# zifuwan/Sigma

Measured on AMD Instinct MI355X. Metric: images/sec fwd+bwd sigma_small 480x640, higher is better.
Workload: dtype f32

## Files before the change

### sigma_amd/csrc/layernorm.hip

```cpp
#include <hip/hip_runtime.h>
#include <stdint.h>

#include "../../include/sigma_ops.h"
#include "scan_device.h"

namespace sigma {

namespace {

__device__ __forceinline__ float wave_allsum(float v) { return wave_sum(v); }

struct LnArgs {
    const float* x; const float* gamma; const float* beta; const float* dy;
    float* y; float* mean; float* rstd; float* dx; float* ws;
    const float* z; float* dz; long z_stride, dz_stride;
    const float* rsc; long rows_per_scale;
    const float* dx_add;
    long M; int C; float eps;
};

__device__ __forceinline__ float sigmoid_f(float v) {
    return __builtin_amdgcn_rcpf(1.0f + __builtin_amdgcn_exp2f(-v * 1.4426950408889634f));
}

template <int NV>
__global__ void __launch_bounds__(256) ln_fwd_kernel(const LnArgs a) {
    const int lane = threadIdx.x & 63;
    const long wave = (long)blockIdx.x * 4 + (threadIdx.x >> 6);
    const long nwaves = (long)gridDim.x * 4;
    const int C = a.C;
    float4 g[NV], b[NV];
#pragma unroll
    for (int j = 0; j < NV; ++j) {
        const int c = lane * 4 + 256 * j;
        g[j] = c < C ? *reinterpret_cast<const float4*>(a.gamma + c) : make_float4(0, 0, 0, 0);
        b[j] = (c < C && a.beta) ? *reinterpret_cast<const float4*>(a.beta + c) : make_float4(0, 0, 0, 0);
    }
    const float inv = 1.0f / (float)C;
    long sb = a.rsc ? wave / a.rows_per_scale : 0, srem = a.rsc ? wave - sb * a.rows_per_scale : 0;
    const bool gatedf = a.z != nullptr;
    auto load_row = [&](long r, float4 (&xv)[NV], float4 (&zv)[NV]) {
        const float* __restrict__ xr = a.x + r * C;
#pragma unroll
        for (int j = 0; j < NV; ++j) {
            const int c = lane * 4 + 256 * j;
            xv[j] = c < C ? *reinterpret_cast<const float4*>(xr + c) : make_float4(0, 0, 0, 0);
            zv[j] = (gatedf && c < C) ? *reinterpret_cast<const float4*>(a.z + r * a.z_stride + c) : make_float4(0, 0, 0, 0);
        }
    };
    constexpr bool kPrefetch = NV <= 2;
    float4 v[NV], zc[NV];
    if (kPrefetch && wave < a.M) load_row(wave, v, zc);
    for (long r = wave; r < a.M; r += nwaves) {
        if (!kPrefetch) load_row(r, v, zc);
        float4 vn[NV], zn[NV];
        const bool more = kPrefetch && r + nwaves < a.M;
        if (more) load_row(r + nwaves, vn, zn);
        float s = 0.0f;
#pragma unroll
        for (int j = 0; j < NV; ++j) s += (v[j].x + v[j].y) + (v[j].z + v[j].w);
        const float mu = wave_allsum(s) * inv;
        float q = 0.0f;
#pragma unroll
        for (int j = 0; j < NV; ++j) {
            const int c = lane * 4 + 256 * j;
            if (c < C) {
                const float dx0 = v[j].x - mu, dx1 = v[j].y - mu, dx2 = v[j].z - mu, dx3 = v[j].w - mu;
                q += (dx0 * dx0 + dx1 * dx1) + (dx2 * dx2 + dx3 * dx3);
            }
        }
        const float rs = rsqrtf(wave_allsum(q) * inv + a.eps);
        float* __restrict__ yr = a.y + r * C;
        float sc = 1.0f;
        if (a.rsc) {
            sc = a.rsc[sb];
            srem += nwaves;
            while (srem >= a.rows_per_scale) { srem -= a.rows_per_scale; ++sb; }
        }
#pragma unroll
        for (int j = 0; j < NV; ++j) {
            const int c = lane * 4 + 256 * j;
            if (c < C) {
                float4 o;
                o.x = (v[j].x - mu) * rs * g[j].x + b[j].x;
                o.y = (v[j].y - mu) * rs * g[j].y + b[j].y;
                o.z = (v[j].z - mu) * rs * g[j].z + b[j].z;
                o.w = (v[j].w - mu) * rs * g[j].w + b[j].w;
                if (gatedf) {
                    const float4 zv = zc[j];
                    o.x *= zv.x * sigmoid_f(zv.x); o.y *= zv.y * sigmoid_f(zv.y);
                    o.z *= zv.z * sigmoid_f(zv.z); o.w *= zv.w * sigmoid_f(zv.w);
                }
                if (a.rsc) { o.x *= sc; o.y *= sc; o.z *= sc; o.w *= sc; }
                *reinterpret_cast<float4*>(yr + c) = o;
            }
        }
        if (lane == 0 && a.mean) { a.mean[r] = mu; a.rstd[r] = rs; }
        if (more) {
#pragma unroll
            for (int j = 0; j < NV; ++j) { v[j] = vn[j]; zc[j] = zn[j]; }
        }
    }
}

template <int NV>
__global__ void __launch_bounds__(256) ln_bwd_kernel(const LnArgs a) {
    const int lane = threadIdx.x & 63;
    const long wave = (long)blockIdx.x * 4 + (threadIdx.x >> 6);
    const long nwaves = (long)gridDim.x * 4;
    const int C = a.C;
    float4 g[NV], dg[NV], db[NV];
#pragma unroll
    for (int j = 0; j < NV; ++j) {
        const int c = lane * 4 + 256 * j;
        g[j] = c < C ? *reinterpret_cast<const float4*>(a.gamma + c) : make_float4(0, 0, 0, 0);
        dg[j] = make_float4(0, 0, 0, 0);
        db[j] = make_float4(0, 0, 0, 0);
    }
    const bool gated = a.z != nullptr;
    const float inv = 1.0f / (float)C;
    long sb = a.rsc ? wave / a.rows_per_scale : 0, srem = a.rsc ? wave - sb * a.rows_per_scale : 0;
    auto load_row = [&](long r, float4 (&xv)[NV], float4 (&gv)[NV], float4 (&zv)[NV], float& mu, float& rs) {
        const float* __restrict__ xr = a.x + r * C;
        const float* __restrict__ gr = a.dy + r * C;
        mu = a.mean[r]; rs = a.rstd[r];
#pragma unroll
        for (int j = 0; j < NV; ++j) {
            const int c = lane * 4 + 256 * j;
            const bool in = c < C;
            xv[j] = in ? *reinterpret_cast<const float4*>(xr + c) : make_float4(0, 0, 0, 0);
            gv[j] = in ? *reinterpret_cast<const float4*>(gr + c) : make_float4(0, 0, 0, 0);
            zv[j] = (gated && in) ? *reinterpret_cast<const float4*>(a.z + r * a.z_stride + c) : make_float4(0, 0, 0, 0);
        }
    };
    float4 bv_[NV];
#pragma unroll
    for (int j = 0; j < NV; ++j) {
        const int c = lane * 4 + 256 * j;
        bv_[j] = (gated && a.beta && c < C) ? *reinterpret_cast<const float4*>(a.beta + c) : make_float4(0, 0, 0, 0);
    }
    constexpr bool kPrefetch = NV <= 2;
    float4 xc[NV], gc[NV], zc[NV];
    float mu = 0.0f, rs = 0.0f;
    if (kPrefetch && wave < a.M) load_row(wave, xc, gc, zc, mu, rs);
    for (long r = wave; r < a.M; r += nwaves) {
        if (!kPrefetch) load_row(r, xc, gc, zc, mu, rs);
        float4 xn[NV], gn[NV], zn[NV];
        float mun = 0.0f, rsn = 0.0f;
        const bool more = kPrefetch && r + nwaves < a.M;
        if (more) load_row(r + nwaves, xn, gn, zn, mun, rsn);
        float sc = 1.0f;
        if (a.rsc) {
            sc = a.rsc[sb];
            srem += nwaves;
            while (srem >= a.rows_per_scale) { srem -= a.rows_per_scale; ++sb; }
        }
        float4 xh[NV], t[NV];
        float s1 = 0.0f, s2 = 0.0f;
#pragma unroll
        for (int j = 0; j < NV; ++j) {
            const int c = lane * 4 + 256 * j;
            if (c < C) {
                const float4 xv = xc[j];
                float4 gv = gc[j];
                if (a.rsc) { gv.x *= sc; gv.y *= sc; gv.z *= sc; gv.w *= sc; }
                xh[j] = make_float4((xv.x - mu) * rs, (xv.y - mu) * rs, (xv.z - mu) * rs, (xv.w - mu) * rs);
                if (gated) {
                    const float4 zv = zc[j];
                    const float4 bv = bv_[j];
                    const float s0 = sigmoid_f(zv.x), s1_ = sigmoid_f(zv.y), s2_ = sigmoid_f(zv.z), s3 = sigmoid_f(zv.w);
                    float4 dzv;
                    dzv.x = gv.x * fmaf(xh[j].x, g[j].x, bv.x) * s0 * fmaf(zv.x, 1.0f - s0, 1.0f);
                    dzv.y = gv.y * fmaf(xh[j].y, g[j].y, bv.y) * s1_ * fmaf(zv.y, 1.0f - s1_, 1.0f);
                    dzv.z = gv.z * fmaf(xh[j].z, g[j].z, bv.z) * s2_ * fmaf(zv.z, 1.0f - s2_, 1.0f);
                    dzv.w = gv.w * fmaf(xh[j].w, g[j].w, bv.w) * s3 * fmaf(zv.w, 1.0f - s3, 1.0f);
                    *reinterpret_cast<float4*>(a.dz + r * a.dz_stride + c) = dzv;
                    gv.x *= zv.x * s0; gv.y *= zv.y * s1_; gv.z *= zv.z * s2_; gv.w *= zv.w * s3;
                }
                t[j] = make_float4(gv.x * g[j].x, gv.y * g[j].y, gv.z * g[j].z, gv.w * g[j].w);
                s1 += (t[j].x + t[j].y) + (t[j].z + t[j].w);
                s2 += (t[j].x * xh[j].x + t[j].y * xh[j].y) + (t[j].z * xh[j].z + t[j].w * xh[j].w);
                dg[j].x += gv.x * xh[j].x; dg[j].y += gv.y * xh[j].y; dg[j].z += gv.z * xh[j].z; dg[j].w += gv.w * xh[j].w;
                db[j].x += gv.x; db[j].y += gv.y; db[j].z += gv.z; db[j].w += gv.w;
            } else {
                xh[j] = make_float4(0, 0, 0, 0);
                t[j] = make_float4(0, 0, 0, 0);
            }
        }
        const float m1 = wave_allsum(s1) * inv, m2 = wave_allsum(s2) * inv;
        float* __restrict__ dr = a.dx + r * C;
        const float* __restrict__ ar = a.dx_add ? a.dx_add + r * C : nullptr;
#pragma unroll
        for (int j = 0; j < NV; ++j) {
            const int c = lane * 4 + 256 * j;
            if (c < C) {
                float4 o;
                o.x = rs * (t[j].x - m1 - xh[j].x * m2);
                o.y = rs * (t[j].y - m1 - xh[j].y * m2);
                o.z = rs * (t[j].z - m1 - xh[j].z * m2);
                o.w = rs * (t[j].w - m1 - xh[j].w * m2);
                if (ar) {
                    const float4 e = *reinterpret_cast<const float4*>(ar + c);
                    o.x += e.x; o.y += e.y; o.z += e.z; o.w += e.w;
                }
                *reinterpret_cast<float4*>(dr + c) = o;
            }
        }
        if (more) {
#pragma unroll
            for (int j = 0; j < NV; ++j) { xc[j] = xn[j]; gc[j] = gn[j]; zc[j] = zn[j]; }
            mu = mun; rs = rsn;
        }
    }
    extern __shared__ float part[];
    const int wv = threadIdx.x >> 6;
#pragma unroll
    for (int j = 0; j < NV; ++j) {
        const int c = lane * 4 + 256 * j;
        if (c < C) {
            *reinterpret_cast<float4*>(part + (wv * 2 + 0) * C + c) = dg[j];
            *reinterpret_cast<float4*>(part + (wv * 2 + 1) * C + c) = db[j];
        }
    }
    __syncthreads();
    float* __restrict__ wrow = a.ws + (long)blockIdx.x * 2 * C;
    for (int i = threadIdx.x * 4; i < 2 * C; i += 1024) {
        const float4 p0 = *reinterpret_cast<const float4*>(part + i), p1 = *reinterpret_cast<const float4*>(part + 2 * C + i);
        const float4 p2 = *reinterpret_cast<const float4*>(part + 4 * C + i), p3 = *reinterpret_cast<const float4*>(part + 6 * C + i);
        *reinterpret_cast<float4*>(wrow + i) = make_float4((p0.x + p1.x) + (p2.x + p3.x), (p0.y + p1.y) + (p2.y + p3.y),
                                                          (p0.z + p1.z) + (p2.z + p3.z), (p0.w + p1.w) + (p2.w + p3.w));
    }
}

__global__ void __launch_bounds__(256) ln_reduce_kernel(const float* __restrict__ ws, float* __restrict__ dgamma,
                                                        float* __restrict__ dbeta, int nwaves, int C) {
    __shared__ float red[16][17];
    const int tx = threadIdx.x & 15, ty = threadIdx.x >> 4;
    const int i = blockIdx.x * 16 + tx;
    const bool live = i < 2 * C;
    const int which = live ? i / C : 0, c = live ? i - which * C : 0;
    const float* __restrict__ col = ws + (long)which * C + c;
    const long stride = 2L * C;
    float a0 = 0.0f, a1 = 0.0f, a2 = 0.0f, a3 = 0.0f;
    if (live) {
        int w = ty;
        for (; w + 48 < nwaves; w += 64) {
            a0 += col[(long)w * stride];
            a1 += col[(long)(w + 16) * stride];
            a2 += col[(long)(w + 32) * stride];
            a3 += col[(long)(w + 48) * stride];
        }
        for (; w < nwaves; w += 16) a0 += col[(long)w * stride];
    }
    red[ty][tx] = (a0 + a1) + (a2 + a3);
    __syncthreads();
    if (ty == 0 && live) {
        float acc = 0.0f;
#pragma unroll
        for (int k = 0; k < 16; ++k) acc += red[k][tx];
        if (which == 0) dgamma[c] = acc;
        else if (dbeta) dbeta[c] = acc;
    }
}

template <typename F>
bool dispatch_nv(int C, F&& f) {
    const int nv = (C + 255) / 256;
    switch (nv) {
        case 1: f(std::integral_constant<int, 1>()); return true;
        case 2: f(std::integral_constant<int, 2>()); return true;
        case 3: f(std::integral_constant<int, 3>()); return true;
        case 4: f(std::integral_constant<int, 4>()); return true;
        case 5: case 6: f(std::integral_constant<int, 6>()); return true;
        case 7: case 8: f(std::integral_constant<int, 8>()); return true;
        default: return false;
    }
}

int grid_blocks(long M, long cap = 2048) {
    long b = (M + 3) / 4;
    if (b > cap) b = cap;
    if (b < 1) b = 1;
    return (int)b;
}
constexpr long kBwdBlocks = 512;
long bwd_blocks(long rows, int C) {
    long cap = (2L << 20) / (8L * C);
    if (cap > 2048) cap = 2048;
    if (cap < kBwdBlocks) cap = kBwdBlocks;
    return cap;
}

template <int NV, bool BWD>
int resident_blocks() {
    static int cached = 0;
    if (cached == 0) {
        int n = 0;
        hipError_t e = BWD ? hipOccupancyMaxActiveBlocksPerMultiprocessor(&n, ln_bwd_kernel<NV>, 256, 8 * 256 * NV * sizeof(float))
                           : hipOccupancyMaxActiveBlocksPerMultiprocessor(&n, ln_fwd_kernel<NV>, 256, 0);
        cached = (e == hipSuccess && n > 0) ? (n > 8 ? 8 : n) : 4;
    }
    return cached;
}

int fwd_grid(long rows, int C) {
    int occ = 8;
    dispatch_nv(C, [&](auto nv) { occ = resident_blocks<decltype(nv)::value, false>(); });
    return grid_blocks(rows, 256L * occ);
}

int bwd_grid(long rows, int C) {
    int occ = 8;
    dispatch_nv(C, [&](auto nv) { occ = resident_blocks<decltype(nv)::value, true>(); });
    long cap = bwd_blocks(rows, C);
    if (cap > 256L * occ) cap = 256L * occ;
    return grid_blocks(rows, cap);
}

bool check(const sigma_layernorm_params* p) {
    return p && p->rows >= 0 && p->channels > 0 && p->channels % 4 == 0 && p->channels <= 2048;
}

}

}

extern "C" {

int sigma_layernorm_bwd_partial_rows(int64_t rows, int32_t channels) {
    return sigma::bwd_grid(rows, channels > 0 ? channels : 4);
}

int sigma_layernorm_fwd(const sigma_layernorm_params* p, void* stream) {
    if (!sigma::check(p)) return SIGMA_OPS_ERR_ARG;
    if (p->rows == 0) return SIGMA_OPS_OK;
    if (!p->x || !p->gamma || !p->y) return SIGMA_OPS_ERR_ARG;
    sigma::LnArgs a{};
    a.x = p->x; a.gamma = p->gamma; a.beta = p->beta; a.y = p->y; a.mean = p->mean; a.rstd = p->rstd;
    a.z = p->gate; a.z_stride = p->gate_row_stride;
    if (p->gate && (p->gate_row_stride % 4 != 0 || p->gate_row_stride < p->channels)) return SIGMA_OPS_ERR_ARG;
    a.rsc = p->row_scale; a.rows_per_scale = p->rows_per_scale;
    if (p->row_scale && p->rows_per_scale <= 0) return SIGMA_OPS_ERR_ARG;
    a.M = p->rows; a.C = p->channels; a.eps = p->eps;
    const int grid = sigma::fwd_grid(p->rows, p->channels);
    hipStream_t s = static_cast<hipStream_t>(stream);
    const bool ok = sigma::dispatch_nv(p->channels, [&](auto nv) {
        hipLaunchKernelGGL(sigma::ln_fwd_kernel<decltype(nv)::value>, dim3(grid), dim3(256), 0, s, a);
    });
    if (!ok) return SIGMA_OPS_ERR_ARG;
    return hipGetLastError() == hipSuccess ? SIGMA_OPS_OK : SIGMA_OPS_ERR_LAUNCH;
}

int sigma_layernorm_bwd(const sigma_layernorm_params* p, void* stream) {
    if (!sigma::check(p)) return SIGMA_OPS_ERR_ARG;
    if (!p->dgamma) return SIGMA_OPS_ERR_ARG;
    hipStream_t s = static_cast<hipStream_t>(stream);
    const int grid = sigma::bwd_grid(p->rows, p->channels);
    if (p->rows > 0) {
        if (!p->x || !p->gamma || !p->dy || !p->mean || !p->rstd || !p->dx || !p->workspace) return SIGMA_OPS_ERR_ARG;
        sigma::LnArgs a{};
        a.x = p->x; a.gamma = p->gamma; a.beta = p->beta; a.dy = p->dy; a.mean = p->mean; a.rstd = p->rstd; a.dx = p->dx;
        a.ws = p->workspace; a.z = p->gate; a.z_stride = p->gate_row_stride; a.dz = p->dgate;
        a.dz_stride = p->dgate_row_stride > 0 ? p->dgate_row_stride : p->channels;
        a.rsc = p->row_scale; a.rows_per_scale = p->rows_per_scale;
        a.dx_add = p->dx_add;
        if (p->dx_add && (reinterpret_cast<uintptr_t>(p->dx_add) & 15)) return SIGMA_OPS_ERR_ARG;
        if (p->row_scale && p->rows_per_scale <= 0) return SIGMA_OPS_ERR_ARG;
        if (p->gate && (!p->dgate || p->gate_row_stride % 4 != 0 || p->gate_row_stride < p->channels || a.dz_stride % 4 != 0 ||
                        a.dz_stride < p->channels))
            return SIGMA_OPS_ERR_ARG;
        a.M = p->rows; a.C = p->channels; a.eps = p->eps;
        const bool ok = sigma::dispatch_nv(p->channels, [&](auto nv) {
            hipLaunchKernelGGL(sigma::ln_bwd_kernel<decltype(nv)::value>, dim3(grid), dim3(256), 8 * p->channels * sizeof(float), s, a);
        });
        if (!ok) return SIGMA_OPS_ERR_ARG;
        if (hipGetLastError() != hipSuccess) return SIGMA_OPS_ERR_LAUNCH;
    }
    const int nw = p->rows > 0 ? grid : 0;
    hipLaunchKernelGGL(sigma::ln_reduce_kernel, dim3((2 * p->channels + 15) / 16), dim3(256), 0, s, p->workspace, p->dgamma,
                       p->dbeta, nw, p->channels);
    return hipGetLastError() == hipSuccess ? SIGMA_OPS_OK : SIGMA_OPS_ERR_LAUNCH;
}

}
```

Measured before the change: 50.89.

## Add two-rows-per-wave LayerNorm kernels for channels up to 128

For channel counts of 128 or fewer, new forward and backward LayerNorm kernels map two rows onto each 64-lane wave, each half-wave handling one row. Reductions use a half-wave DPP sum, and the backward kernel software-prefetches the next batch of rows. The goal is to stop leaving most lanes idle on narrow rows, as the one-row-per-wave kernel does. Grid sizing and the per-block gamma/beta partial reduction are adjusted for the doubled row count per wave, at the cost of extra kernel variants and more complex indexing.

```diff
diff --git a/sigma_amd/csrc/layernorm.hip b/sigma_amd/csrc/layernorm.hip
--- a/sigma_amd/csrc/layernorm.hip
+++ b/sigma_amd/csrc/layernorm.hip
@@ -232,6 +232,221 @@
     }
 }
 
+__device__ __forceinline__ float half_allsum(float v, int lane) {
+#define SIGMA_ADD(CTRL, MASK) v += dpp_take<CTRL, MASK>(0.0f, v);
+    SIGMA_ADD(DPP_ROW_SHR1, 0xF)
+    SIGMA_ADD(DPP_ROW_SHR2, 0xF)
+    SIGMA_ADD(DPP_ROW_SHR4, 0xF)
+    SIGMA_ADD(DPP_ROW_SHR8, 0xF)
+    SIGMA_ADD(DPP_ROW_BCAST15, 0xA)
+#undef SIGMA_ADD
+    const float lo = __builtin_bit_cast(float, __builtin_amdgcn_readlane(__builtin_bit_cast(int, v), 31));
+    const float hi = __builtin_bit_cast(float, __builtin_amdgcn_readlane(__builtin_bit_cast(int, v), 63));
+    return lane < 32 ? lo : hi;
+}
+
+template <int R, bool PF, bool GATED>
+__global__ void __launch_bounds__(256) ln_fwd_rows_kernel(const LnArgs a) {
+    const int lane = threadIdx.x & 63;
+    const int c = (lane & 31) * 4, half = lane >> 5;
+    const long wave = (long)blockIdx.x * 4 + __builtin_amdgcn_readfirstlane((int)(threadIdx.x >> 6));
+    const long nwaves = (long)gridDim.x * 4;
+    const int C = a.C;
+    const bool live = c < C;
+    const float4 g = live ? *reinterpret_cast<const float4*>(a.gamma + c) : make_float4(0, 0, 0, 0);
+    const float4 b = (live && a.beta) ? *reinterpret_cast<const float4*>(a.beta + c) : make_float4(0, 0, 0, 0);
+    const float inv = 1.0f / (float)C;
+    const long step = nwaves * 2;
+    long sb = a.rsc ? wave * 2 / a.rows_per_scale : 0, srem = a.rsc ? wave * 2 - sb * a.rows_per_scale : 0;
+    auto load_pass = [&](long i0, float4 (&xv)[R], float4 (&zv)[R]) {
+#pragma unroll
+        for (int k = 0; k < R; ++k) {
+            const long r = ((i0 + k) * nwaves + wave) * 2 + half;
+            const bool in = live && r < a.M;
+            xv[k] = in ? *reinterpret_cast<const float4*>(a.x + r * C + c) : make_float4(0, 0, 0, 0);
+            if (GATED) zv[k] = in ? *reinterpret_cast<const float4*>(a.z + r * a.z_stride + c) : make_float4(0, 0, 0, 0);
+        }
+    };
+    float4 v[R], zc[R];
+    if (PF && wave * 2 < a.M) load_pass(0, v, zc);
+    for (long i0 = 0; (i0 * nwaves + wave) * 2 < a.M; i0 += R) {
+        if (!PF) load_pass(i0, v, zc);
+        float4 vn[R], zn[R];
+        const bool more = PF && ((i0 + R) * nwaves + wave) * 2 < a.M;
+        if (more) load_pass(i0 + R, vn, zn);
+        float mu[R], q[R], rs[R];
+#pragma unroll
+        for (int k = 0; k < R; ++k)
+            mu[k] = half_allsum(0.0f + ((v[k].x + v[k].y) + (v[k].z + v[k].w)), lane) * inv;
+#pragma unroll
+        for (int k = 0; k < R; ++k) {
+            q[k] = 0.0f;
+            if (live) {
+                const float dx0 = v[k].x - mu[k], dx1 = v[k].y - mu[k], dx2 = v[k].z - mu[k], dx3 = v[k].w - mu[k];
+                q[k] += (dx0 * dx0 + dx1 * dx1) + (dx2 * dx2 + dx3 * dx3);
+            }
+        }
+#pragma unroll
+        for (int k = 0; k < R; ++k) rs[k] = rsqrtf(half_allsum(q[k], lane) * inv + a.eps);
+#pragma unroll
+        for (int k = 0; k < R; ++k) {
+            const long r = ((i0 + k) * nwaves + wave) * 2 + half;
+            const bool ok = r < a.M;
+            float sc = 1.0f;
+            if (a.rsc) {
+                if (ok) sc = a.rsc[sb + (srem + half >= a.rows_per_scale ? 1 : 0)];
+                srem += step;
+                while (srem >= a.rows_per_scale) { srem -= a.rows_per_scale; ++sb; }
+            }
+            if (live && ok) {
+                float4 o;
+                o.x = (v[k].x - mu[k]) * rs[k] * g.x + b.x;
+                o.y = (v[k].y - mu[k]) * rs[k] * g.y + b.y;
+                o.z = (v[k].z - mu[k]) * rs[k] * g.z + b.z;
+                o.w = (v[k].w - mu[k]) * rs[k] * g.w + b.w;
+                if (GATED) {
+                    const float4 zv = zc[k];
+                    o.x *= zv.x * sigmoid_f(zv.x); o.y *= zv.y * sigmoid_f(zv.y);
+                    o.z *= zv.z * sigmoid_f(zv.z); o.w *= zv.w * sigmoid_f(zv.w);
+                }
+                if (a.rsc) { o.x *= sc; o.y *= sc; o.z *= sc; o.w *= sc; }
+                *reinterpret_cast<float4*>(a.y + r * C + c) = o;
+            }
+            if (c == 0 && ok && a.mean) { a.mean[r] = mu[k]; a.rstd[r] = rs[k]; }
+        }
+        if (more) {
+#pragma unroll
+            for (int k = 0; k < R; ++k) { v[k] = vn[k]; if (GATED) zc[k] = zn[k]; }
+        }
+    }
+}
+
+template <int R, bool PF, bool GATED>
+__global__ void __launch_bounds__(256) ln_bwd_rows_kernel(const LnArgs a) {
+    const int lane = threadIdx.x & 63;
+    const int c = (lane & 31) * 4, half = lane >> 5;
+    const int wv = __builtin_amdgcn_readfirstlane((int)(threadIdx.x >> 6));
+    const long wave = (long)blockIdx.x * 4 + wv;
+    const long nwaves = (long)gridDim.x * 4;
+    const int C = a.C;
+    const bool live = c < C;
+    const float4 g = live ? *reinterpret_cast<const float4*>(a.gamma + c) : make_float4(0, 0, 0, 0);
+    const float4 bv = (GATED && a.beta && live) ? *reinterpret_cast<const float4*>(a.beta + c) : make_float4(0, 0, 0, 0);
+    float4 dg = make_float4(0, 0, 0, 0), db = make_float4(0, 0, 0, 0);
+    const float inv = 1.0f / (float)C;
+    const long step = nwaves * 2;
+    long sb = a.rsc ? wave * 2 / a.rows_per_scale : 0, srem = a.rsc ? wave * 2 - sb * a.rows_per_scale : 0;
+    const bool early_add = !GATED && a.dx_add != nullptr;
+    auto load_pass = [&](long i0, float4 (&xv)[R], float4 (&gv)[R], float4 (&zv)[R], float (&mu)[R], float (&rs)[R]) {
+#pragma unroll
+        for (int k = 0; k < R; ++k) {
+            const long r = ((i0 + k) * nwaves + wave) * 2 + half;
+            const bool ok = r < a.M, in = live && ok;
+            mu[k] = ok ? a.mean[r] : 0.0f;
+            rs[k] = ok ? a.rstd[r] : 0.0f;
+            xv[k] = in ? *reinterpret_cast<const float4*>(a.x + r * C + c) : make_float4(0, 0, 0, 0);
+            gv[k] = in ? *reinterpret_cast<const float4*>(a.dy + r * C + c) : make_float4(0, 0, 0, 0);
+            if (GATED) zv[k] = in ? *reinterpret_cast<const float4*>(a.z + r * a.z_stride + c) : make_float4(0, 0, 0, 0);
+            else zv[k] = (in && early_add) ? *reinterpret_cast<const float4*>(a.dx_add + r * C + c) : make_float4(0, 0, 0, 0);
+        }
+    };
+    float4 xc[R], gc[R], zc[R];
+    float mu[R], rs[R];
+    if (PF && wave * 2 < a.M) load_pass(0, xc, gc, zc, mu, rs);
+    for (long i0 = 0; (i0 * nwaves + wave) * 2 < a.M; i0 += R) {
+        if (!PF) load_pass(i0, xc, gc, zc, mu, rs);
+        float4 xn[R], gn[R], zn[R];
+        float mun[R], rsn[R];
+        const bool more = PF && ((i0 + R) * nwaves + wave) * 2 < a.M;
+        if (more) load_pass(i0 + R, xn, gn, zn, mun, rsn);
+        float4 xh[R], t[R];
+        float s1[R], s2[R], m1[R], m2[R];
+#pragma unroll
+        for (int k = 0; k < R; ++k) {
+            const long r = ((i0 + k) * nwaves + wave) * 2 + half;
+            const bool ok = r < a.M;
+            float sc = 1.0f;
+            if (a.rsc) {
+                if (ok) sc = a.rsc[sb + (srem + half >= a.rows_per_scale ? 1 : 0)];
+                srem += step;
+                while (srem >= a.rows_per_scale) { srem -= a.rows_per_scale; ++sb; }
+            }
+            s1[k] = 0.0f; s2[k] = 0.0f;
+            if (live && ok) {
+                const float4 xv = xc[k];
+                float4 gv = gc[k];
+                if (a.rsc) { gv.x *= sc; gv.y *= sc; gv.z *= sc; gv.w *= sc; }
+                xh[k] = make_float4((xv.x - mu[k]) * rs[k], (xv.y - mu[k]) * rs[k], (xv.z - mu[k]) * rs[k], (xv.w - mu[k]) * rs[k]);
+                if (GATED) {
+                    const float4 zv = zc[k];
+                    const float s0 = sigmoid_f(zv.x), s1_ = sigmoid_f(zv.y), s2_ = sigmoid_f(zv.z), s3 = sigmoid_f(zv.w);
+                    float4 dzv;
+                    dzv.x = gv.x * fmaf(xh[k].x, g.x, bv.x) * s0 * fmaf(zv.x, 1.0f - s0, 1.0f);
+                    dzv.y = gv.y * fmaf(xh[k].y, g.y, bv.y) * s1_ * fmaf(zv.y, 1.0f - s1_, 1.0f);
+                    dzv.z = gv.z * fmaf(xh[k].z, g.z, bv.z) * s2_ * fmaf(zv.z, 1.0f - s2_, 1.0f);
+                    dzv.w = gv.w * fmaf(xh[k].w, g.w, bv.w) * s3 * fmaf(zv.w, 1.0f - s3, 1.0f);
+                    *reinterpret_cast<float4*>(a.dz + r * a.dz_stride + c) = dzv;
+                    gv.x *= zv.x * s0; gv.y *= zv.y * s1_; gv.z *= zv.z * s2_; gv.w *= zv.w * s3;
+                }
+                t[k] = make_float4(gv.x * g.x, gv.y * g.y, gv.z * g.z, gv.w * g.w);
+                s1[k] += (t[k].x + t[k].y) + (t[k].z + t[k].w);
+                s2[k] += (t[k].x * xh[k].x + t[k].y * xh[k].y) + (t[k].z * xh[k].z + t[k].w * xh[k].w);
+                dg.x += gv.x * xh[k].x; dg.y += gv.y * xh[k].y; dg.z += gv.z * xh[k].z; dg.w += gv.w * xh[k].w;
+                db.x += gv.x; db.y += gv.y; db.z += gv.z; db.w += gv.w;
+            } else {
+                xh[k] = make_float4(0, 0, 0, 0);
+                t[k] = make_float4(0, 0, 0, 0);
+            }
+        }
+#pragma unroll
+        for (int k = 0; k < R; ++k) m1[k] = half_allsum(s1[k], lane) * inv;
+#pragma unroll
+        for (int k = 0; k < R; ++k) m2[k] = half_allsum(s2[k], lane) * inv;
+#pragma unroll
+        for (int k = 0; k < R; ++k) {
+            const long r = ((i0 + k) * nwaves + wave) * 2 + half;
+            if (live && r < a.M) {
+                float4 o;
+                o.x = rs[k] * (t[k].x - m1[k] - xh[k].x * m2[k]);
+                o.y = rs[k] * (t[k].y - m1[k] - xh[k].y * m2[k]);
+                o.z = rs[k] * (t[k].z - m1[k] - xh[k].z * m2[k]);
+                o.w = rs[k] * (t[k].w - m1[k] - xh[k].w * m2[k]);
+                if (early_add) {
+                    const float4 e = zc[k];
+                    o.x += e.x; o.y += e.y; o.z += e.z; o.w += e.w;
+                } else if (GATED && a.dx_add) {
+                    const float4 e = *reinterpret_cast<const float4*>(a.dx_add + r * C + c);
+                    o.x += e.x; o.y += e.y; o.z += e.z; o.w += e.w;
+                }
+                *reinterpret_cast<float4*>(a.dx + r * C + c) = o;
+            }
+        }
+        if (more) {
+#pragma unroll
+            for (int k = 0; k < R; ++k) { xc[k] = xn[k]; gc[k] = gn[k]; zc[k] = zn[k]; mu[k] = mun[k]; rs[k] = rsn[k]; }
+        }
+    }
+    extern __shared__ float part[];
+    if (live) {
+        *reinterpret_cast<float4*>(part + ((wv * 2 + half) * 2 + 0) * C + c) = dg;
+        *reinterpret_cast<float4*>(part + ((wv * 2 + half) * 2 + 1) * C + c) = db;
+    }
+    __syncthreads();
+    float* __restrict__ wrow = a.ws + (long)blockIdx.x * 2 * C;
+    for (int i = threadIdx.x * 4; i < 2 * C; i += 1024) {
+        float4 acc[2];
+#pragma unroll
+        for (int h = 0; h < 2; ++h) {
+            const float* __restrict__ ph = part + h * 8 * C + i;
+            const float4 p0 = *reinterpret_cast<const float4*>(ph), p1 = *reinterpret_cast<const float4*>(ph + 2 * C);
+            const float4 p2 = *reinterpret_cast<const float4*>(ph + 4 * C), p3 = *reinterpret_cast<const float4*>(ph + 6 * C);
+            acc[h] = make_float4((p0.x + p1.x) + (p2.x + p3.x), (p0.y + p1.y) + (p2.y + p3.y),
+                                 (p0.z + p1.z) + (p2.z + p3.z), (p0.w + p1.w) + (p2.w + p3.w));
+        }
+        *reinterpret_cast<float4*>(wrow + i) = make_float4(acc[0].x + acc[1].x, acc[0].y + acc[1].y, acc[0].z + acc[1].z, acc[0].w + acc[1].w);
+    }
+}
+
 __global__ void __launch_bounds__(256) ln_reduce_kernel(const float* __restrict__ ws, float* __restrict__ dgamma,
                                                         float* __restrict__ dbeta, int nwaves, int C) {
     __shared__ float red[16][17];
@@ -291,6 +506,12 @@
     return cap;
 }
 
+constexpr int kRowsMaxC = 128;
+using LnKernel = void (*)(const LnArgs);
+inline LnKernel fwd_rows_kernel(bool gated) { return gated ? ln_fwd_rows_kernel<2, false, true> : ln_fwd_rows_kernel<2, false, false>; }
+inline LnKernel bwd_rows_kernel(bool gated) { return gated ? ln_bwd_rows_kernel<2, true, true> : ln_bwd_rows_kernel<2, true, false>; }
+inline size_t rows_lds_bytes(int C) { return 16 * (size_t)C * sizeof(float); }
+
 template <int NV, bool BWD>
 int resident_blocks() {
     static int cached = 0;
@@ -302,17 +523,45 @@
     }
     return cached;
 }
+template <bool BWD>
+int rows_resident_blocks() {
+    static int cached = 0;
+    if (cached == 0) {
+        int occ = BWD ? 3 : 8;
+        for (int gated = 0; gated < 2; ++gated) {
+            int n = 0;
+            hipError_t e = hipOccupancyMaxActiveBlocksPerMultiprocessor(&n, BWD ? bwd_rows_kernel(gated != 0) : fwd_rows_kernel(gated != 0),
+                                                                        256, BWD ? rows_lds_bytes(kRowsMaxC) : 0);
+            n = (e == hipSuccess && n > 0) ? n : 4;
+            if (n < occ) occ = n;
+        }
+        cached = occ;
+    }
+    return cached;
+}
+
+int rows_grid_blocks(long M, long cap) {
+    long b = (M + 7) / 8;
+    if (b > cap) b = cap;
+    if (b < 1) b = 1;
+    return (int)b;
+}
 
 int fwd_grid(long rows, int C) {
+    if (C <= kRowsMaxC) return rows_grid_blocks(rows, 256L * rows_resident_blocks<false>());
     int occ = 8;
     dispatch_nv(C, [&](auto nv) { occ = resident_blocks<decltype(nv)::value, false>(); });
     return grid_blocks(rows, 256L * occ);
 }
 
 int bwd_grid(long rows, int C) {
+    long cap = bwd_blocks(rows, C);
+    if (C <= kRowsMaxC) {
+        const long res = 256L * rows_resident_blocks<true>();
+        return rows_grid_blocks(rows, cap < res ? cap : res);
+    }
     int occ = 8;
     dispatch_nv(C, [&](auto nv) { occ = resident_blocks<decltype(nv)::value, true>(); });
-    long cap = bwd_blocks(rows, C);
     if (cap > 256L * occ) cap = 256L * occ;
     return grid_blocks(rows, cap);
 }
@@ -344,10 +593,14 @@
     a.M = p->rows; a.C = p->channels; a.eps = p->eps;
     const int grid = sigma::fwd_grid(p->rows, p->channels);
     hipStream_t s = static_cast<hipStream_t>(stream);
-    const bool ok = sigma::dispatch_nv(p->channels, [&](auto nv) {
-        hipLaunchKernelGGL(sigma::ln_fwd_kernel<decltype(nv)::value>, dim3(grid), dim3(256), 0, s, a);
-    });
-    if (!ok) return SIGMA_OPS_ERR_ARG;
+    if (p->channels <= sigma::kRowsMaxC) {
+        hipLaunchKernelGGL(sigma::fwd_rows_kernel(p->gate != nullptr), dim3(grid), dim3(256), 0, s, a);
+    } else {
+        const bool ok = sigma::dispatch_nv(p->channels, [&](auto nv) {
+            hipLaunchKernelGGL(sigma::ln_fwd_kernel<decltype(nv)::value>, dim3(grid), dim3(256), 0, s, a);
+        });
+        if (!ok) return SIGMA_OPS_ERR_ARG;
+    }
     return hipGetLastError() == hipSuccess ? SIGMA_OPS_OK : SIGMA_OPS_ERR_LAUNCH;
 }
 
@@ -370,10 +623,14 @@
                         a.dz_stride < p->channels))
             return SIGMA_OPS_ERR_ARG;
         a.M = p->rows; a.C = p->channels; a.eps = p->eps;
-        const bool ok = sigma::dispatch_nv(p->channels, [&](auto nv) {
-            hipLaunchKernelGGL(sigma::ln_bwd_kernel<decltype(nv)::value>, dim3(grid), dim3(256), 8 * p->channels * sizeof(float), s, a);
-        });
-        if (!ok) return SIGMA_OPS_ERR_ARG;
+        if (p->channels <= sigma::kRowsMaxC) {
+            hipLaunchKernelGGL(sigma::bwd_rows_kernel(p->gate != nullptr), dim3(grid), dim3(256), sigma::rows_lds_bytes(p->channels), s, a);
+        } else {
+            const bool ok = sigma::dispatch_nv(p->channels, [&](auto nv) {
+                hipLaunchKernelGGL(sigma::ln_bwd_kernel<decltype(nv)::value>, dim3(grid), dim3(256), 8 * p->channels * sizeof(float), s, a);
+            });
+            if (!ok) return SIGMA_OPS_ERR_ARG;
+        }
         if (hipGetLastError() != hipSuccess) return SIGMA_OPS_ERR_LAUNCH;
     }
     const int nw = p->rows > 0 ? grid : 0;
```

Result: no change. 51.14 (median of 6 runs) (+0.5%).
